# GG1991/macroc

Measured on AMD Instinct MI355X. Metric: Newton-iter DOF/s (assembly+CG) at 256^3 grid per GPU; SpMV achieved HBM GB/s, higher is better.
Workload: dtype f64

## Files before the change

### include/macroc_amd.h

```cpp
#ifndef MACROC_AMD_H
#define MACROC_AMD_H

#include <stddef.h>
#include <stdint.h>

#ifdef __cplusplus
extern "C" {
#endif

#define MCX_COMM_ID_BYTES 128

#define MCX_ABI_VERSION 3

enum { MCX_BC_BENDING = 0, MCX_BC_CIRCLE = 1 };

enum {
  MCX_KSP_CONVERGED_ITERATING = 0,
  MCX_KSP_CONVERGED_RTOL = 2,
  MCX_KSP_CONVERGED_ATOL = 3,
  MCX_KSP_DIVERGED_ITS = -3,
  MCX_KSP_DIVERGED_DTOL = -4,
  MCX_KSP_DIVERGED_INDEFINITE_PC = -8,
  MCX_KSP_DIVERGED_NANORINF = -9,
  MCX_KSP_DIVERGED_INDEFINITE_MAT = -10
// ... 56 lines not shown
  int64_t vi_exc_nodes;
  int64_t split_escapes;
  int64_t st_listed;
} mcx_info;

typedef struct {
  double strains_ms, homogenize_ms, residual_ms, jacobian_ms, solve_ms, update_ms;
  int64_t spmv_launches;
  double spmv_ms_total;
  int64_t spmv_bytes_per_launch;
  int64_t cg_vec_bytes_per_iter;
} mcx_timing;

const char* mcx_last_error(void);
const char* mcx_version(void);
int mcx_abi_version(void);

void mcx_default_opts(mcx_opts* o);
int mcx_parse_args(mcx_opts* o, int argc, const char* const* argv);

int mcx_comm_unique_id(void* id );

int mcx_plan(const mcx_opts* o, int rank, int nranks, mcx_info* info);
int mcx_plan_halo(const mcx_opts* o, int rank, int nranks, int* nnbr, int* nbr_rank, int64_t* send_cnt,
                  int64_t* recv_cnt, int64_t* send_nat, int64_t* recv_nat, int64_t* nsend, int64_t* nrecv);

int mcx_init(const mcx_opts* o, int rank, int nranks, const void* comm_id, void** ctx);
int mcx_local_group_create(int nranks, int device, void** group);
int mcx_local_group_destroy(void* group);
int mcx_local_group_barrier(void* group, int rank);
int mcx_init_local(const mcx_opts* o, int rank, void* group, void** ctx);
int mcx_finalize(void* ctx);
int mcx_get_info(void* ctx, mcx_info* info);
int mcx_comm_info(void* ctx, int* comm_ranks, int* comm_rank, int* device);

int mcx_material_set(void* ctx, int id, double E, double nu, double Sy, double Ka, int type);

typedef struct {
  void (*set_strain3)(int gpi, double* strain);
  void (*homogenize)(void);
  void (*get_stress3)(int gpi, double* stress);
  void (*get_ctan3)(int gpi, double* ctan);
  void (*update_vars)(void);
  int (*get_non_linear_gps)(void);
  double (*get_f_trial_max)(void);
} mcx_micropp_api;

typedef struct {
  int64_t nelem;
  int64_t ngp;
  const double* eps;
  double* sig;
  double* ctan;
  void* stream;
} mcx_gp_batch;

typedef struct {
  int (*homogenize)(void* user, const mcx_gp_batch* batch);
  int (*update_vars)(void* user);
  int (*nonlinear_stats)(void* user, int64_t* n_nonlinear, double* f_trial_max);
  void* user;
} mcx_device_law;

int mcx_set_micropp(void* ctx, const mcx_micropp_api* api);
int mcx_set_device_law(void* ctx, const mcx_device_law* law);
int mcx_set_gp_stress(void* ctx, const double* host );
// ... 58 lines not shown
```

### macroc_amd/__init__.py

```python
import ctypes as C
import os

import numpy as np

_HERE = os.path.dirname(os.path.abspath(__file__))
LIB_PATH = os.path.join(_HERE, "libmacroc_amd.so")
COMM_ID_BYTES = 128
ABI_VERSION = 3

BC_BENDING, BC_CIRCLE = 0, 1
KSP_REASONS = {2: "CONVERGED_RTOL", 3: "CONVERGED_ATOL", -3: "DIVERGED_ITS", -4: "DIVERGED_DTOL",
               -8: "DIVERGED_INDEFINITE_PC", -9: "DIVERGED_NANORINF", -10: "DIVERGED_INDEFINITE_MAT"}

EXPORTS = [
    "mcx_last_error", "mcx_version", "mcx_abi_version", "mcx_comm_info", "mcx_default_opts", "mcx_parse_args", "mcx_comm_unique_id", "mcx_plan", "mcx_plan_halo", "mcx_init",
    "mcx_local_group_create", "mcx_local_group_destroy", "mcx_local_group_barrier", "mcx_init_local",
    "mcx_finalize", "mcx_get_info", "mcx_material_set", "mcx_get_displacement", "mcx_zero_u", "mcx_apply_bc_u",
    "mcx_set_strains", "mcx_homogenize", "mcx_assembly_res", "mcx_assembly_jac", "mcx_solve", "mcx_update_u", "mcx_update_vars",
    "mcx_get_nonlinear_stats", "mcx_reduce_nonlinear", "mcx_calc_force", "mcx_write_vtu",
    "mcx_time_step", "mcx_get_u", "mcx_set_u", "mcx_get_b", "mcx_get_du", "mcx_get_strain", "mcx_get_stress",
    "mcx_owned_dofs", "mcx_dump_csr", "mcx_dump_dirichlet", "mcx_spmv", "mcx_get_ksp_history",
    "mcx_set_timing", "mcx_get_timing", "mcx_synchronize", "mcx_set_option", "mcx_time_spmv",
    "mcx_set_micropp", "mcx_set_device_law", "mcx_set_gp_stress", "mcx_set_gp_ctan", "mcx_get_gp_strain",
    "mcx_micro_get_ctan", "mcx_micro_get_phase",
    "mcx_get_gp_ctan", "mcx_micro_nl_get_info", "mcx_micro_nl_get_pool", "mcx_apply_args",
    "mcx_pc_apply", "mcx_pc_mg_info", "mcx_pc_mg_dump_csr",
]

LAWS = {"elastic": 0, "plastic": 1, "external": 2, "micro": 3, "micro_nl": 4}


class Opts(C.Structure):
    _fields_ = [
        ("NX", C.c_int64), ("NY", C.c_int64), ("NZ", C.c_int64),
        ("px", C.c_int), ("py", C.c_int), ("pz", C.c_int),
        ("lx", C.c_double), ("ly", C.c_double), ("lz", C.c_double),
        ("dt", C.c_double), ("final_time", C.c_double),
        ("ts", C.c_int), ("vtu_freq", C.c_int), ("bc_type", C.c_int), ("rad", C.c_double),
        ("newton_max_its", C.c_int), ("newton_min_tol", C.c_double), ("newton_rel_tol", C.c_double),
        ("ksp_rtol", C.c_double), ("ksp_abstol", C.c_double), ("ksp_dtol", C.c_double),
        ("ksp_max_it", C.c_int), ("micro_n", C.c_int), ("micro_type", C.c_int),
        ("micro_mat_1", C.c_double * 4), ("micro_mat_2", C.c_double * 4),
        ("device", C.c_int), ("ksp_monitor", C.c_int), ("mat_type", C.c_int), ("mat_law", C.c_int),
        ("mat_aij_split", C.c_int),
        ("mat_aij_vi", C.c_int),
        ("mat_vi_fma", C.c_int),
    ]


class Info(C.Structure):
    _fields_ = [
        ("NX", C.c_int64), ("NY", C.c_int64), ("NZ", C.c_int64),
        ("px", C.c_int), ("py", C.c_int), ("pz", C.c_int), ("rank", C.c_int), ("nranks", C.c_int),
        ("xs", C.c_int64), ("ys", C.c_int64), ("zs", C.c_int64), ("nx", C.c_int64), ("ny", C.c_int64), ("nz", C.c_int64),
        ("Xs", C.c_int64), ("Ys", C.c_int64), ("Zs", C.c_int64), ("Nx", C.c_int64), ("Ny", C.c_int64), ("Nz", C.c_int64),
        ("ndofs_global", C.c_int64), ("ndofs_local", C.c_int64), ("dof_offset", C.c_int64),
        ("nnz_local", C.c_int64), ("nnz_global", C.c_int64), ("nelem_local", C.c_int64), ("nelem_ext", C.c_int64),
        ("dx", C.c_double), ("dy", C.c_double), ("dz", C.c_double), ("wg", C.c_double),
        ("device_bytes", C.c_int64), ("device", C.c_int), ("storage", C.c_int), ("split_slots", C.c_int),
# ... 43 lines not shown

_LIB = None


class MacrocError(RuntimeError):
    pass


def lib():
    global _LIB
    if _LIB is not None:
        return _LIB
    if not os.path.exists(LIB_PATH):
        raise MacrocError(f"{LIB_PATH} not built: run `make` (or __graft_entry__.build())")
    L = C.CDLL(LIB_PATH)
    if L.mcx_abi_version() != ABI_VERSION:
        raise MacrocError(f"{LIB_PATH}: ABI {L.mcx_abi_version()}, this mirror needs {ABI_VERSION}: rebuild (`make`)")
    vp, d, i64 = C.c_void_p, C.POINTER(C.c_double), C.POINTER(C.c_int64)
    L.mcx_last_error.restype = C.c_char_p
    L.mcx_version.restype = C.c_char_p
    L.mcx_default_opts.argtypes = [C.POINTER(Opts)]
    L.mcx_parse_args.argtypes = [C.POINTER(Opts), C.c_int, C.POINTER(C.c_char_p)]
    L.mcx_comm_unique_id.argtypes = [C.c_void_p]
    L.mcx_init.argtypes = [C.POINTER(Opts), C.c_int, C.c_int, C.c_void_p, C.POINTER(C.c_void_p)]
    L.mcx_plan.argtypes = [C.POINTER(Opts), C.c_int, C.c_int, C.POINTER(Info)]
    L.mcx_plan_halo.argtypes = [C.POINTER(Opts), C.c_int, C.c_int, C.POINTER(C.c_int), C.POINTER(C.c_int),
                                i64, i64, i64, i64, i64, i64]
    L.mcx_local_group_create.argtypes = [C.c_int, C.c_int, C.POINTER(C.c_void_p)]
    L.mcx_local_group_destroy.argtypes = [vp]
    L.mcx_local_group_barrier.argtypes = [vp, C.c_int]
    L.mcx_init_local.argtypes = [C.POINTER(Opts), C.c_int, vp, C.POINTER(C.c_void_p)]
    L.mcx_finalize.argtypes = [vp]
    L.mcx_get_info.argtypes = [vp, C.POINTER(Info)]
    L.mcx_comm_info.argtypes = [vp, C.POINTER(C.c_int), C.POINTER(C.c_int), C.POINTER(C.c_int)]
    L.mcx_material_set.argtypes = [vp, C.c_int, C.c_double, C.c_double, C.c_double, C.c_double, C.c_int]
    L.mcx_get_displacement.argtypes = [vp, C.c_int]
    L.mcx_get_displacement.restype = C.c_double
    L.mcx_apply_bc_u.argtypes = [vp, C.c_double]
    for fn in ("mcx_zero_u", "mcx_set_strains", "mcx_homogenize", "mcx_assembly_jac", "mcx_update_u",
               "mcx_synchronize", "mcx_update_vars"):
        getattr(L, fn).argtypes = [vp]
    L.mcx_assembly_res.argtypes = [vp, d]
    L.mcx_solve.argtypes = [vp, C.POINTER(C.c_int), d, C.POINTER(C.c_int)]
    L.mcx_time_step.argtypes = [vp, C.c_int, C.POINTER(C.c_int), d, C.POINTER(C.c_int), d]
    for fn in ("mcx_get_u", "mcx_set_u", "mcx_get_b", "mcx_get_du", "mcx_get_strain", "mcx_get_stress"):
        getattr(L, fn).argtypes = [vp, d]
    L.mcx_owned_dofs.argtypes = [vp, i64, i64]
    L.mcx_get_nonlinear_stats.argtypes = [vp, i64, d]
    L.mcx_reduce_nonlinear.argtypes = [vp, i64, i64, d]
    L.mcx_calc_force.argtypes = [vp, d]
    L.mcx_write_vtu.argtypes = [vp, C.c_char_p]
    L.mcx_dump_csr.argtypes = [vp, i64, i64, d]
    L.mcx_dump_dirichlet.argtypes = [vp, i64, i64]
    L.mcx_spmv.argtypes = [vp, d, d]
    L.mcx_get_ksp_history.argtypes = [vp, d, i64]
    L.mcx_set_timing.argtypes = [vp, C.c_int]
    L.mcx_get_timing.argtypes = [vp, C.POINTER(Timing)]
    L.mcx_set_option.argtypes = [vp, C.c_char_p, C.c_double]
    L.mcx_apply_args.argtypes = [vp, C.c_int, C.POINTER(C.c_char_p)]
    L.mcx_time_spmv.argtypes = [vp, C.c_int, d]
    L.mcx_set_micropp.argtypes = [vp, C.POINTER(MicroppApi)]
    L.mcx_set_device_law.argtypes = [vp, C.POINTER(DeviceLaw)]
    ip = C.POINTER(C.c_int)
    L.mcx_micro_nl_get_info.argtypes = [vp, ip, ip, ip, d]
    L.mcx_micro_nl_get_pool.argtypes = [vp, i64, i64, i64]
    for fn in ("mcx_set_gp_stress", "mcx_set_gp_ctan", "mcx_get_gp_strain", "mcx_get_gp_ctan"):
# ... 132 lines not shown

    def apply_bc_on_u(self, U):
        _check(lib().mcx_apply_bc_u(self._ctx, float(U)), "apply_bc_on_u")

    def set_strains(self):
        _check(lib().mcx_set_strains(self._ctx), "set_strains")

    def homogenize(self):
        _check(lib().mcx_homogenize(self._ctx), "micropp_C_homogenize")

    def material_set(self, mid, E, nu, Sy=1e4, Ka=1e7, typ=1):
        _check(lib().mcx_material_set(self._ctx, mid, E, nu, Sy, Ka, typ), "micropp_C_material_set")

    def assembly_res(self):
        nrm = C.c_double()
        _check(lib().mcx_assembly_res(self._ctx, C.byref(nrm)), "assembly_res")
        return nrm.value

    def assembly_jac(self):
        _check(lib().mcx_assembly_jac(self._ctx), "assembly_jac")

    def solve_Ax(self):
        its, rn, reason = C.c_int(), C.c_double(), C.c_int()
        _check(lib().mcx_solve(self._ctx, C.byref(its), C.byref(rn), C.byref(reason)), "solve_Ax")
        return its.value, rn.value, reason.value

    def update_u(self):
        _check(lib().mcx_update_u(self._ctx), "VecAXPY(u,1,du)")

    def update_vars(self):
        _check(lib().mcx_update_vars(self._ctx), "micropp_C_update_vars")

    def get_info(self):
        inf = Info()
        _check(lib().mcx_get_info(self._ctx, C.byref(inf)), "mcx_get_info")
        return inf.as_dict()

    def comm_info(self):
        n, r, d = C.c_int(), C.c_int(), C.c_int()
        _check(lib().mcx_comm_info(self._ctx, C.byref(n), C.byref(r), C.byref(d)), "mcx_comm_info")
        return n.value, r.value, d.value

    def nonlinear_stats(self):
        n, f = C.c_int64(), C.c_double()
        _check(lib().mcx_get_nonlinear_stats(self._ctx, C.byref(n), C.byref(f)), "nonlinear_stats")
        return n.value, f.value

    def reduce_nonlinear(self):
        nl, nt, f = C.c_int64(), C.c_int64(), C.c_double()
        _check(lib().mcx_reduce_nonlinear(self._ctx, C.byref(nl), C.byref(nt), C.byref(f)), "reduce_nonlinear")
        return nl.value, nt.value, f.value

    def write_vtu(self, prefix):
        _check(lib().mcx_write_vtu(self._ctx, str(prefix).encode()), "write_vtu")

    def calc_force(self):
        f = C.c_double()
        _check(lib().mcx_calc_force(self._ctx, C.byref(f)), "calc_force")
        return f.value

    def time_step(self, time_s):
        k = max(self.opts.newton_max_its, 1)
        nits = C.c_int()
        res, kr = np.zeros(k), np.zeros(k)
        ki = (C.c_int * k)()
        _check(lib().mcx_time_step(self._ctx, int(time_s), C.byref(nits), _dp(res), ki, _dp(kr)), "time_step")
        n = nits.value
        return dict(newton_its=n, res=res[: n + 1 if n < k else n].tolist(), ksp_its=list(ki)[:n],
                    ksp_rnorm=kr[:n].tolist())
# ... 163 lines not shown
```

### macroc_amd/csrc/api.cpp

```cpp
#include <algorithm>
#include <cmath>
#include <cstdio>
#include <cstdlib>
#include <cstring>
#include <string>
#include <unordered_map>
#include <vector>

#include "mcx_internal.h"

namespace mcx {

static thread_local std::string g_err;
void set_error(const std::string& s) { g_err = s; }

int exc_return(const char* fn, const char* what) {
  try {
    g_err = std::string(fn) + ": internal exception: " + what;
  } catch (...) {
  }
  return MCX_EXC;
}

static const std::string g_test_throw = [] {
// ... 579 lines not shown
  }
  in->nelem_local = cnt[0] * cnt[1] * cnt[2];
  in->nelem_ext = g.nelem;
  in->dx = g.dx;
  in->dy = c.dy;
  in->dz = g.dz;
  in->wg = g.wg;
  in->device_bytes = c.device_bytes;
  in->device = c.device;
  in->storage = c.fmt;
  in->split_slots = c.fmt == FMT_SPLIT ? c.dsl.L : 0;
  in->split_bits = c.fmt == FMT_SPLIT ? (c.dsl.wide ? 32 : 16) : 0;
  in->vi_values = c.fmt == FMT_VI ? c.vi_n : 0;
  in->vi_bits = c.fmt == FMT_VI ? c.vi_bits : 0;
  in->vi_blocks = c.fmt == FMT_VI && c.vi_block ? c.vi_nblocks : 0;
  in->vi_exc_nodes = c.fmt == FMT_VI && c.vi_block ? c.vi_nexc : 0;
  in->split_escapes = c.fmt == FMT_SPLIT && c.dsl.esc ? c.dsl.nesc : 0;
  in->st_listed = c.device >= 0 && st_used(c) ? c.st_n : -1;
  if (c.device >= 0) spmv_tile(c, &in->spmv_tx, &in->spmv_ty, &in->spmv_kc);
  in->ex0 = g.ex0;
  in->ey0 = g.ey0;
  in->ez0 = g.ez0;
  in->nex = g.nex;
  in->ney = g.ney;
  in->nez = g.nez;
}


int mcx_get_info(void* ctx, mcx_info* in) try {
  MCX_ENTRY();
  GUARD(ctx);
  CTX(ctx);
  fill_info(c, in);
  return 0;
} MCX_CATCH

int mcx_comm_info(void* ctx, int* comm_ranks, int* comm_rank, int* device) try {
  MCX_ENTRY();
  GUARD(ctx);
  CTX(ctx);
  int n = 1, r = 0, d = c.device;
  if (c.lg) {
    n = c.lg->nranks;
    r = c.rank;
  } else if (int rc = comm_query(c, &n, &r, &d)) {
    return rc;
  }
  if (comm_ranks) *comm_ranks = n;
  if (comm_rank) *comm_rank = r;
  if (device) *device = d;
  return 0;
} MCX_CATCH

int mcx_plan(const mcx_opts* o, int rank, int nranks, mcx_info* in) try {
  MCX_ENTRY();
  if (!o || !in || nranks < 1 || rank < 0 || rank >= nranks) {
    set_error("mcx_plan: bad arguments");
    return 1;
  }
  Ctx c;
  c.o = *o;
  c.rank = rank;
  c.nranks = nranks;
  c.device = -1;
  int rc = setup_decomposition(c);
  if (rc) return rc;
// ... 1557 lines not shown
      set_error("vi_st_faces: partials buffer too small");
      return (c.st_ok || c.st_pending) && build_st(c) ? 1 : 2;
    }
    return 0;
  }
  if (!std::strcmp(name, "vi_st_pair")) {
    const int old = c.vi_st_pair;
    c.vi_st_pair = value != 0.;
    if (!partials_fit(c)) {
      c.vi_st_pair = old;
      set_error("vi_st_pair: partials buffer too small");
      return 2;
    }
    return 0;
  }
  if (!std::strcmp(name, "vi_st_fstream")) {
    c.vi_st_fstream = value != 0.;
    return 0;
  }
  if (!std::strcmp(name, "vi_st_l16")) {
    if (!(value == -1. || value == 0. || value == 1.)) {
      set_error("vi_st_l16: -1 (by the list's length), 0 or 1");
      return 1;
    }
    const int old = c.vi_st_l16;
    c.vi_st_l16 = (int)value;
    if (!partials_fit(c)) {
      c.vi_st_l16 = old;
      set_error("vi_st_l16: partials buffer too small");
      return 2;
    }
    return 0;
  }
  if (!std::strcmp(name, "vi_st_pf")) {
    if (!(value == 1. || value == 2. || value == 3.)) {
      set_error("vi_st_pf: 1 or 2");
      return 1;
    }
    c.vi_st_pf = (int)value;
    return 0;
  }
  if (!std::strcmp(name, "vi_st_ty")) {
    if (!(value == 8. || value == 16.)) {
      set_error("vi_st_ty: 8 or 16");
      return 1;
    }
    const int old = c.vi_st_ty;
    c.vi_st_ty = (int)value;
    if (!partials_fit(c)) {
      c.vi_st_ty = old;
      set_error("vi_st_ty: partials buffer too small");
      return 2;
    }
    return 0;
  }
  if (!std::strcmp(name, "vi_st_tail")) {
    const int old = c.vi_st_tail;
    c.vi_st_tail = value != 0.;
    if (!partials_fit(c)) {
      c.vi_st_tail = old;
      set_error("vi_st_tail: partials buffer too small");
      return 2;
    }
    return 0;
  }
  if (!std::strcmp(name, "vi_st")) {
// ... 224 lines not shown
```

### macroc_amd/csrc/kernels.hip

```cpp
#include <algorithm>
#include <cstring>
#include <cmath>

#include "mcx_internal.h"

namespace mcx {

__constant__ double cB[8][6][24];

static constexpr int TPB = 256;

__device__ __forceinline__ void node_ijk(const Geo& g, int n, int& i, int& j, int& k) {
  i = n % g.nx;
  int t = n / g.nx;
  j = t % g.ny;
  k = t / g.ny;
}

__device__ __forceinline__ int pad_of(const Geo& g, int i, int j, int k) {
  return (i + 1) + (j + 1) * g.PX + (k + 1) * g.PX * g.PY;
}

__device__ __forceinline__ int u_of(const Geo& g, int i, int j, int k) {
  return 64 + i + (j + 1) * g.UX + (k + 1) * g.UXY;
}

__host__ __device__ inline int dirichlet_mask(const Geo& g, int gi, int gj, int gk) {
  if (g.bc_type == MCX_BC_CIRCLE) {
    if (gj == 0 && (gi == 0 || gi == g.NX - 1 || gk == 0 || gk == g.NZ - 1)) return 7;
    if (gj == g.NY - 1) {
      double x = g.lx / 2. - ((double)gi * g.dx + g.dx / 2.);
      double z = g.lz / 2. - ((double)gk * g.dz + g.dz / 2.);
      if ((x * x + z * z) < (g.rad * g.rad)) return 2;
    }
    return 0;
  }
  if (g.bc_type == MCX_BC_BENDING) return (gi == 0 || gi == g.NX - 1) ? 7 : 0;
// ... 4210 lines not shown
    if (more && !NOSTAGE) {
      __syncthreads();
#pragma unroll
      for (int m = 0; m < NL; m++) {
        const int e = me + m * T;
        if (e < PLANE) {
          xs[(k + 3 - k0 + 1) & 3][e] = PF2 ? cur[0][m] : xr[0][m];
          xs[(k + 4 - k0 + 1) & 3][e] = PF2 ? cur[1][m] : xr[1][m];
        }
      }
      __syncthreads();
    }
  };
  if (PF2) {
    for (int k = k0; k < k1; k += 4) {
      step(k, pfa, pfb);
      if (k + 2 < k1) step(k + 2, pfb, pfa);
    }
  } else {
    for (int k = k0; k < k1; k += 2) step(k, pfa, pfb);
  }
  if (TAIL) {
    __syncthreads();
    st_faces(g, sf, coef, slot, x, y, dot, &xs[0][0]);
    st_tail<T>(g, list, (int64_t)b * cnt / gridDim.x, (int64_t)(b + 1) * cnt / gridDim.x, I, bdict, exc, x, y,
               reinterpret_cast<double2*>(&xs[0][0]), dot);
  }
  if (DOT) {
    const double s = block_sum<T>(dot, sh);
    if (threadIdx.x == 0) part[blockIdx.x] = s;
  }
}

template <bool DOT, bool GATED, bool L16 = true>
__global__ __launch_bounds__(SFP_T) void k_spmv_face(Geo g, StFaces sf, const double* __restrict__ coef,
                                                   const unsigned* __restrict__ slot, const double* __restrict__ x,
                                                   double* __restrict__ y, double* __restrict__ part,
                                                   const CgState* __restrict__ cg, const int* __restrict__ list,
                                                   int64_t cnt, const u32x4* __restrict__ I,
                                                   const double* __restrict__ bdict, const double* __restrict__ exc,
                                                   int nd = VI_MAX) {
  static_assert(SFP_N >= VI_MAX * VIB_STRIDE, "the dictionary fits the patch's LDS");
  __shared__ __attribute__((aligned(16))) double S[SFP_N];
  __shared__ double sh[SFP_T / 64];
  if (GATED && cg->reason) return;
  double dot = 0.;
  constexpr int LPB = L16 ? SFP_T / ST16 : SFP_T;
  const int64_t NLB = (cnt + LPB - 1) / LPB;
  if ((int64_t)blockIdx.x >= NLB) {
    const SfPatch q = sf_patch(g, sf, blockIdx.x - NLB);
    sf_stage(g, q, x, S, threadIdx.x);
    __syncthreads();
    sf_rows(g, q, coef, slot, S, y, dot, threadIdx.x);
  } else {
    const int64_t lo = (int64_t)blockIdx.x * LPB;
    if (L16) st_tail16<SFP_T>(g, list, lo, min(cnt, lo + LPB), I, bdict, exc, x, y, reinterpret_cast<double2*>(S), dot, nd);
    else st_tail<SFP_T>(g, list, lo, min(cnt, lo + LPB), I, bdict, exc, x, y, reinterpret_cast<double2*>(S), dot, nd);
  }
  if (DOT) {
    const double sm = block_sum<SFP_T>(dot, sh);
    if (threadIdx.x == 0) part[blockIdx.x] = sm;
  }
}

constexpr int SP_RLP = 198;

// ... 1537 lines not shown
  return (face_enum(c.g).n + TPB - 1) / TPB;
}

bool fusep(const Ctx& c);
bool st_fusep(const Ctx& c);

static bool st_auto(const Ctx& c) {
  return c.g.nown >= ST_MIN_NODES || (c.vi_nexc > 0 && c.vi_nexc * 10 <= (int64_t)c.g.nown);
}

bool st_used(const Ctx& c) {
  int tx, ty;
  vis_shape(c, tx, ty);
  return st_wanted(c) && c.st_ok && c.fmt == FMT_VI && c.vi_block && vi_staged(c) && c.vi_fma && c.vi_uni && c.vi_patch &&
         tx == 64 && (!fusep(c) || st_fusep(c));
}

bool st_fusep(const Ctx& c) { return c.vi_st_pair && !c.vi_st_tail; }

static bool sp_used(const Ctx& c) { return st_used(c) && c.vi_st_pair && !c.vi_st_tail; }

static ZTiling sp_tiling(const Ctx& c) {
  const int ty = c.vi_st_ty;
  ZTiling t;
  t.ntx = (c.g.nx + 63) / 64;
  t.nty = (c.g.ny + ty - 1) / ty;
  const int tiles = t.ntx * t.nty, want = c.spmv_zblocks > 0 ? c.spmv_zblocks : c.g.ncu * (16 / ty);
  t.nzc = std::max(1, std::min(c.g.nz, (want + tiles - 1) / tiles));
  t.kc = (c.g.nz + t.nzc - 1) / t.nzc;
  t.nzc = (c.g.nz + t.kc - 1) / t.kc;
  return t;
}

static bool st_l16(const Ctx& c) {
  return c.vi_st_l16 > 0 || (c.vi_st_l16 < 0 && (int64_t)ST16 * c.st_n * 2 <= (int64_t)c.g.ncu * 1024);
}

static int64_t stface_blocks(const Ctx& c) {
  const int lpb = st_l16(c) ? SFP_T / ST16 : SFP_T;
  return st_used(c) && !c.vi_st_tail ? c.st_faces.u[6] + (c.st_n + lpb - 1) / lpb : 0;
}

static int64_t exc_blocks(const Ctx& c) {
  if (!(c.fmt == FMT_VI && c.vi_block && c.vi_nexc && vi_staged(c) && c.vi_exc_kernel) || st_used(c)) return 0;
  return (c.vi_nexc + TPB - 1) / TPB;
}

int64_t spmv_nparts(const Ctx& c) {
  if (c.fmt == FMT_SPLIT && c.dsl.dense) return node_blocks(c);
  return spmv_grid_blocks(c) + faces_blocks(c) + exc_blocks(c) + stface_blocks(c);
}

bool partials_fit(const Ctx& c) {
  return std::max(spmv_nparts(c), node_blocks(c)) + 32 <= c.partials_cap / 2;
}

bool st_wanted(const Ctx& c) { return c.vi_st == 1 || (c.vi_st < 0 && st_auto(c)); }

int upload_constants(Ctx& c) {
  double B[8][6][24];
  compute_B_table(B);
  MCX_HIP(hipMemcpyToSymbol(HIP_SYMBOL(cB), B, sizeof(B)));
  return 0;
}

void launch_apply_bc_u(Ctx& c, double U) {
// ... 792 lines not shown
    }
  return true;
}

template <bool DV, bool GV, int D>
static void sp_dbg1(Ctx& c, int nb, const double* xpad, double* y, const ZTiling& zt) {
  if (c.vi_st_ty == 16)
    hipLaunchKernelGGL((k_spmv_sp<DV, GV, 16, false, D>), dim3(nb), dim3(1024), 0, c.stream, c.g, c.st_coef,
                       c.st_mask, c.st_npx, c.st_npy, xpad, y, c.partials, c.cg, zt);
  else
    hipLaunchKernelGGL((k_spmv_sp<DV, GV, 8, false, D>), dim3(nb), dim3(512), 0, c.stream, c.g, c.st_coef,
                       c.st_mask, c.st_npx, c.st_npy, xpad, y, c.partials, c.cg, zt);
}
template <bool DV, bool GV>
static void sp_dbg(Ctx& c, int nb, const double* xpad, double* y, const ZTiling& zt) {
  switch (zt.dbg) {
    case 1: sp_dbg1<DV, GV, 1>(c, nb, xpad, y, zt); break;
    case 2: sp_dbg1<DV, GV, 2>(c, nb, xpad, y, zt); break;
    case 3: sp_dbg1<DV, GV, 3>(c, nb, xpad, y, zt); break;
    case 4: sp_dbg1<DV, GV, 4>(c, nb, xpad, y, zt); break;
    case 8: sp_dbg1<DV, GV, 8>(c, nb, xpad, y, zt); break;
    case 12: sp_dbg1<DV, GV, 12>(c, nb, xpad, y, zt); break;
    case 44: sp_dbg1<DV, GV, 44>(c, nb, xpad, y, zt); break;
    case 1024: sp_dbg1<DV, GV, 1024>(c, nb, xpad, y, zt); break;
    case 36: sp_dbg1<DV, GV, 36>(c, nb, xpad, y, zt); break;
    case 40: sp_dbg1<DV, GV, 40>(c, nb, xpad, y, zt); break;
    case 32: sp_dbg1<DV, GV, 32>(c, nb, xpad, y, zt); break;
    case 35: sp_dbg1<DV, GV, 35>(c, nb, xpad, y, zt); break;
    default: sp_dbg1<DV, GV, 0>(c, nb, xpad, y, zt); break;
  }
}

void launch_spmv(Ctx& c, const double* xpad, double* y, bool dot, bool gated) {
  const int nb = (int)spmv_grid_blocks(c);
  const SpmvTiling tl = spmv_tiling(c.g, c.spmv_subl);
  if (c.fmt == FMT_VI && c.vi_block) {
    const u32x4* I = reinterpret_cast<const u32x4*>(c.vi_idx);
    if (vi_staged(c)) {
      ZTiling zt = vis_tiling(c);
      zt.dbg = c.split_dbg;
      zt.wmap = c.vi_wmap;
      zt.xlist = c.vi_exc_list;
      zt.xskip = exc_blocks(c) > 0;
      zt.ypair = c.vi_ypair && (c.g.nx % 2) == 0;
      int tx, ty;
      vis_shape(c, tx, ty);
      if (st_used(c)) {
        if (sp_used(c)) {
          const int dbg = zt.dbg;
          zt = sp_tiling(c);
          zt.dbg = dbg;
        }
        StFaces sfv = c.st_faces;
        int64_t stn = c.st_n, nbfa = stface_blocks(c);
        if (c.face_dbg && nbfa) {
          if (c.face_dbg & 1) stn = 0;
          if (c.face_dbg & 2) {
            const int64_t d = sfv.u[2];
            for (int q = 1; q < 7; q++) sfv.u[q] = std::max<int64_t>(0, sfv.u[q] - d);
          }
          if (c.face_dbg & 4)
            for (int q = 3; q < 7; q++) sfv.u[q] = sfv.u[2];
          const int lpb = st_l16(c) ? SFP_T / ST16 : SFP_T;
          nbfa = sfv.u[6] + (stn + lpb - 1) / lpb;
        }
        double* pf = c.partials + nb;
        const int ndict = c.vi_nblocks > 0 ? c.vi_nblocks : VI_MAX;
#define MCX_SP_DBG(DV, GV) sp_dbg<DV, GV>(c, nb, xpad, y, zt)
#define MCX_ST(DV, GV)                                                                                             \
  do {                                                                                                            \
    const bool fs = nbfa && !c.vi_st_tail && fstream_ok(c);        \
    hipStream_t fst = fs ? c.f_stream : c.stream;                                                                 \
    if (fs) (void)hipEventRecord(c.ev_fx, c.stream);                                                              \
    if (c.vi_st_tail)                                                                                             \
      hipLaunchKernelGGL((k_spmv_st<DV, GV, true>), dim3(nb), dim3(1024), 0, c.stream, c.g, c.st_coef, c.st_mask,   \
                         c.st_npx, c.st_npy, xpad, y, c.partials, c.cg, zt, c.st_list, c.st_n, I, c.vi_bdict,     \
                         c.vi_exc, c.st_slot, c.st_faces);                                                        \
    else if (c.vi_st_pair && zt.dbg > 0)                                                                        \
      MCX_SP_DBG(DV, GV);                                                                                         \
    else if (c.vi_st_pair && c.vi_st_ty == 16)                                                                    \
      hipLaunchKernelGGL((k_spmv_sp<DV, GV, 16>), dim3(nb), dim3(1024), 0, c.stream, c.g, c.st_coef, c.st_mask,     \
                         c.st_npx, c.st_npy, xpad, y, c.partials, c.cg, zt);                                      \
    else if (c.vi_st_pair)                                                                                        \
      hipLaunchKernelGGL((k_spmv_sp<DV, GV, 8>), dim3(nb), dim3(512), 0, c.stream, c.g, c.st_coef, c.st_mask,       \
                         c.st_npx, c.st_npy, xpad, y, c.partials, c.cg, zt);                                      \
    else if (c.vi_st_pf == 3)                                                                                     \
      hipLaunchKernelGGL((k_spmv_st<DV, GV, false, false, true>), dim3(nb), dim3(1024), 0, c.stream, c.g,            \
                         c.st_coef, c.st_mask, c.st_npx, c.st_npy, xpad, y, c.partials, c.cg, zt);                \
    else if (c.vi_st_pf == 2)                                                                                     \
      hipLaunchKernelGGL((k_spmv_st<DV, GV, false, true>), dim3(nb), dim3(1024), 0, c.stream, c.g, c.st_coef,       \
                         c.st_mask, c.st_npx, c.st_npy, xpad, y, c.partials, c.cg, zt);                           \
    else                                                                                                          \
      hipLaunchKernelGGL((k_spmv_st<DV, GV>), dim3(nb), dim3(1024), 0, c.stream, c.g, c.st_coef, c.st_mask,         \
                         c.st_npx, c.st_npy, xpad, y, c.partials, c.cg, zt);                                      \
    if (fs) (void)hipStreamWaitEvent(fst, c.ev_fx, 0);                                                            \
    if (nbfa && st_l16(c))                                                                                        \
      hipLaunchKernelGGL((k_spmv_face<DV, GV>), dim3((unsigned)nbfa), dim3(SFP_T), 0, fst, c.g, sfv,                \
                         c.st_coef, c.st_slot, xpad, y, pf, c.cg, c.st_list, stn, I, c.vi_bdict, c.vi_exc, ndict); \
    else if (nbfa)                                                                                                \
      hipLaunchKernelGGL((k_spmv_face<DV, GV, false>), dim3((unsigned)nbfa), dim3(SFP_T), 0, fst, c.g,              \
                         sfv, c.st_coef, c.st_slot, xpad, y, pf, c.cg, c.st_list, stn, I, c.vi_bdict,   \
                         c.vi_exc, ndict);                                                                        \
    if (fs) {                                                                                                     \
      (void)hipEventRecord(c.ev_fd, fst);                                                                         \
      (void)hipStreamWaitEvent(c.stream, c.ev_fd, 0);                                                             \
    }                                                                                                             \
  } while (0)
        if (dot && gated) MCX_ST(true, true);
        else if (dot) MCX_ST(true, false);
        else MCX_ST(false, false);
#undef MCX_ST
#undef MCX_SP_DBG
        return;
      }
#define MCX_VIBM(TXV, TYV, XVV, UV, PV, ...)                                                                          \
  do {                                                                                                             \
    if (dot && gated)                                                                                              \
      hipLaunchKernelGGL((k_spmv_vibm<true, true, TXV, TYV, XVV, UV, PV, ##__VA_ARGS__>), dim3(nb), dim3(1024), 0,        \
                         c.stream, c.g, I, c.vi_bdict, xpad, y, c.partials, c.cg, zt);                             \
    else if (dot)                                                                                                  \
      hipLaunchKernelGGL((k_spmv_vibm<true, false, TXV, TYV, XVV, UV, PV, ##__VA_ARGS__>), dim3(nb), dim3(1024), 0,       \
                         c.stream, c.g, I, c.vi_bdict, xpad, y, c.partials, c.cg, zt);                             \
    else                                                                                                           \
      hipLaunchKernelGGL((k_spmv_vibm<false, false, TXV, TYV, XVV, UV, PV, ##__VA_ARGS__>), dim3(nb), dim3(1024), 0,      \
// ... 829 lines not shown
```

### macroc_amd/csrc/mcx_internal.h

```cpp
#pragma once

#include <hip/hip_runtime.h>

#include <cstdint>
#include <string>
#include <vector>

#include "../../include/macroc_amd.h"

namespace mcx {

constexpr int NGP = 8, NPE = 8, NVOI = 6;
constexpr int NSLOT = 243;
constexpr int NPAIR = 122;
constexpr int GROUP = 64;
constexpr int USLOT = 123;
constexpr int UPAIR = 62;

void set_error(const std::string& s);

struct Geo {
  int NX, NY, NZ;
  int xs, ys, zs;
  int nx, ny, nz;
// ... 252 lines not shown
  double* h_vib_dict = nullptr;
  int vib_onepass = 1;
  unsigned char* elem_plain = nullptr;
  double* cref = nullptr;
  unsigned* vi_xslot = nullptr;
  int* vi_xlist = nullptr;
  unsigned* vi_xcnt = nullptr;
  double* vi_exc = nullptr;
  int64_t vi_exc_bytes = 0;
  int64_t vi_nexc = 0;
  bool plain_ke = false;
  int vi_exc_max = 300;
  double* ke_uni = nullptr;
  int aij_vi = 1;
  int vi_fma = 1;
  int vi_patch = 1;
  int vi_ring3 = 0;
  int vi_exc_list = VI_EXC_LIST;
  int vi_wmap = 1;
  int vi_tx = 0;
  int vi_uni = 1;
  int vi_ypair = 0;
  int cg_ublocks = 0;
  int vi_lg = 2;
  int cg_p2d = 0;
  int vi_lg_exc = 1;
  int vi_st = -1;
  int vi_st_faces = 1;
  int vi_st_l16 = -1;
  int vi_st_pf = 1;
  int vi_st_ty = 16;
  int vi_st_pair = 0;
  int vi_st_tail = 0;
  double* st_coef = nullptr;
  unsigned* st_ids = nullptr;
  unsigned* st_slot = nullptr;
  int* st_list = nullptr;
  unsigned* st_cnt = nullptr;
  unsigned long long* st_mask = nullptr;
  int64_t st_mask_bytes = 0, st_n = 0;
  int st_npx = 0, st_npy = 0;
  bool st_ok = false;
  bool st_pending = false;
  unsigned st_fm = 0;
  StFaces st_faces = {};
  int vi_exc_kernel = 1;
  int vi_wdesc = 1;
  unsigned* wd = nullptr;
  int64_t wd_bytes = 0;
  bool wd_ok = false;
  int wd_npx = 0, wd_npy = 0;
  int64_t wd_blocks_fma = 0, wd_blocks_exact = 0, wd_blocks_two = 0;
  int vi_xread = 1;
  int vi_stage = -1;
  bool vi_declined = false;
  int fmt = FMT_V;
  bool assembled = false;
  int aij_split = 1;
  int split_maxq = 4;
  int split_dense = 1;
  bool split_declined = false;
  int split_dbg = 0;
  int face_dbg = 0;
  int split_wide = 0;
  int split_tx = 0;
  int split_ty = 0;
// ... 211 lines not shown
```

Baseline: 22.35 million.

## Stage stencil SpMV x-planes into LDS via buffer-load-to-LDS DMA ring

Adds a variant of the structured-stencil SpMV kernel that uses buffer_load ... lds (direct global-to-LDS loads) to fill a 5-slot ring of staged x planes. Two z-planes are processed per iteration with prefetch of upcoming planes, so x loads skip VGPRs and overlap with FMA work. The variant is picked by default when eligibility checks on padding alignment, PX parity and option settings pass, and it is exposed through a query function. The cost is heavier LDS use (close to the 160KB limit) and extra barriers, which may lower occupancy.

```diff
diff --git a/include/macroc_amd.h b/include/macroc_amd.h
--- a/include/macroc_amd.h
+++ b/include/macroc_amd.h
@@ -112,6 +112,7 @@
 int mcx_init_local(const mcx_opts* o, int rank, void* group, void** ctx);
 int mcx_finalize(void* ctx);
 int mcx_get_info(void* ctx, mcx_info* info);
+int mcx_get_st_dma(void* ctx, int* on);
 int mcx_comm_info(void* ctx, int* comm_ranks, int* comm_rank, int* device);
 
 int mcx_material_set(void* ctx, int id, double E, double nu, double Sy, double Ka, int type);
diff --git a/macroc_amd/__init__.py b/macroc_amd/__init__.py
--- a/macroc_amd/__init__.py
+++ b/macroc_amd/__init__.py
@@ -24,7 +24,7 @@
     "mcx_set_micropp", "mcx_set_device_law", "mcx_set_gp_stress", "mcx_set_gp_ctan", "mcx_get_gp_strain",
     "mcx_micro_get_ctan", "mcx_micro_get_phase",
     "mcx_get_gp_ctan", "mcx_micro_nl_get_info", "mcx_micro_nl_get_pool", "mcx_apply_args",
-    "mcx_pc_apply", "mcx_pc_mg_info", "mcx_pc_mg_dump_csr",
+    "mcx_pc_apply", "mcx_pc_mg_info", "mcx_pc_mg_dump_csr", "mcx_get_st_dma",
 ]
 
 LAWS = {"elastic": 0, "plastic": 1, "external": 2, "micro": 3, "micro_nl": 4}
@@ -134,6 +134,7 @@
     L.mcx_init_local.argtypes = [C.POINTER(Opts), C.c_int, vp, C.POINTER(C.c_void_p)]
     L.mcx_finalize.argtypes = [vp]
     L.mcx_get_info.argtypes = [vp, C.POINTER(Info)]
+    L.mcx_get_st_dma.argtypes = [vp, C.POINTER(C.c_int)]
     L.mcx_comm_info.argtypes = [vp, C.POINTER(C.c_int), C.POINTER(C.c_int), C.POINTER(C.c_int)]
     L.mcx_material_set.argtypes = [vp, C.c_int, C.c_double, C.c_double, C.c_double, C.c_double, C.c_int]
     L.mcx_get_displacement.argtypes = [vp, C.c_int]
@@ -332,9 +333,10 @@
         _check(lib().mcx_update_vars(self._ctx), "micropp_C_update_vars")
 
     def get_info(self):
-        inf = Info()
+        inf, on = Info(), C.c_int()
         _check(lib().mcx_get_info(self._ctx, C.byref(inf)), "mcx_get_info")
-        return inf.as_dict()
+        _check(lib().mcx_get_st_dma(self._ctx, C.byref(on)), "mcx_get_st_dma")
+        return dict(inf.as_dict(), st_dma=on.value)
 
     def comm_info(self):
         n, r, d = C.c_int(), C.c_int(), C.c_int()
diff --git a/macroc_amd/csrc/api.cpp b/macroc_amd/csrc/api.cpp
--- a/macroc_amd/csrc/api.cpp
+++ b/macroc_amd/csrc/api.cpp
@@ -635,6 +635,14 @@
   GUARD(ctx);
   CTX(ctx);
   fill_info(c, in);
+  return 0;
+} MCX_CATCH
+
+int mcx_get_st_dma(void* ctx, int* on) try {
+  MCX_ENTRY();
+  GUARD(ctx);
+  CTX(ctx);
+  if (on) *on = c.st_dma_last;
   return 0;
 } MCX_CATCH
 
@@ -2258,6 +2266,14 @@
     }
     return 0;
   }
+  if (!std::strcmp(name, "vi_st_dma")) {
+    if (!(value == -1. || value == 0. || value == 1.)) {
+      set_error("vi_st_dma: -1 (where eligible), 0 or 1");
+      return 1;
+    }
+    c.vi_st_dma = (int)value;
+    return 0;
+  }
   if (!std::strcmp(name, "vi_st_pf")) {
     if (!(value == 1. || value == 2. || value == 3.)) {
       set_error("vi_st_pf: 1 or 2");
diff --git a/macroc_amd/csrc/kernels.hip b/macroc_amd/csrc/kernels.hip
--- a/macroc_amd/csrc/kernels.hip
+++ b/macroc_amd/csrc/kernels.hip
@@ -3,6 +3,7 @@
 #include <cmath>
 
 #include "mcx_internal.h"
+#include "st_dma_map.h"
 
 namespace mcx {
 
@@ -4279,6 +4280,155 @@
   }
 }
 
+typedef __attribute__((address_space(3))) void st_lds_void;
+__device__ __forceinline__ void st_dma16(__amdgpu_buffer_rsrc_t r, double* dst, unsigned voff) {
+  __builtin_amdgcn_raw_ptr_buffer_load_lds(r, (st_lds_void*)dst, 16, voff, 0, 0, 0);
+}
+
+template <bool DOT, bool GATED>
+__global__ __launch_bounds__(1024) void k_spmv_st_dma(Geo g, const double* __restrict__ coef,
+                                                      const unsigned long long* __restrict__ mask, int npx, int npy,
+                                                      const double* __restrict__ x, double* __restrict__ y,
+                                                      double* __restrict__ part, const CgState* __restrict__ cg,
+                                                      ZTiling zt, int sft) {
+  constexpr int TX = ST_DMA_TX, TY = ST_DMA_TY, T = TX * TY, RL = ST_DMA_RL, SLOT = ST_DMA_SLOT, NS = ST_DMA_SLOTS;
+  static_assert(RL == vibm_rl<TX, true>() && T == 64 * ST_DMA_WAVES, "k_spmv_st's staged plane");
+  constexpr int S9 = NS * SLOT, SH = S9 + 27, NLDS = SH + T / 64;
+  static_assert(NLDS * sizeof(double) <= 160 * 1024, "the 5-slot ring fits a CU's LDS");
+  __shared__ __attribute__((aligned(16))) double L[NLDS];
+  if (GATED && cg->reason) return;
+  const int b = blockIdx.x;
+  const int xcd = b & 7, t8 = b >> 3;
+  const int slab = (zt.nty + 7) >> 3;
+  const int ty0 = xcd * slab;
+  const int nty_here = min(slab, zt.nty - ty0);
+  const int per = max(nty_here, 0) * zt.ntx * zt.nzc;
+  const int me = threadIdx.x;
+  double dot = 0.;
+  if (t8 >= per) {
+    if (DOT) {
+      const double s = block_sum<T>(dot, &L[SH]);
+      if (threadIdx.x == 0) part[blockIdx.x] = s;
+    }
+    return;
+  }
+  const int txi = t8 % zt.ntx, r8 = t8 / zt.ntx;
+  const int tyi = ty0 + r8 % nty_here, zc = r8 / nty_here;
+  const int i0 = txi * TX, j0 = tyi * TY;
+  const int k0 = zc * zt.kc, k1 = min(g.nz, k0 + zt.kc);
+  const int wv = __builtin_amdgcn_readfirstlane(me >> 6), ln = me & 63;
+  if (me < 27) L[S9 + me] = coef[me * VIB_STRIDE + 8];
+  const int px = wv & 3, py = wv >> 2;
+  const int lx = px * 16 + (ln & 15), ly = py * 4 + (ln >> 4);
+  const int i = i0 + lx, j = j0 + ly;
+  const bool inxy = i < g.nx && j < g.ny;
+  const int PX = g.PX, PXY = g.PX * g.PY;
+  const int gpx = __builtin_amdgcn_readfirstlane((i0 >> 4) + px), gpy = __builtin_amdgcn_readfirstlane((j0 >> 2) + py);
+  const bool wvin = gpx < npx && gpy < npy;
+  const int len = 3 * min(TX + 2, g.nx + 2 - i0);
+  const int rows = min(TY + 2, g.ny + 2 - j0);
+  const int pc0 = st_dma_piece(wv, 0), pc1 = st_dma_piece(wv, 1);
+  const bool has1 = st_dma_piece_ok(pc1);
+  const unsigned src0 = st_dma_src(pc0, ln, i0, j0, PX, len, rows, sft);
+  const unsigned src1 = has1 ? st_dma_src(pc1, ln, i0, j0, PX, len, rows, sft) : ST_DMA_OOB;
+  auto dma = [&](int p, int so) {
+    const __amdgpu_buffer_rsrc_t rx = sp_rsrc(x + (int64_t)(p + 1) * PXY * 3 - st_dma_rec_lead(sft) / 8,
+                                              p > g.nz ? 0 : st_dma_rec_bytes(PXY, sft));
+    st_dma16(rx, &L[so + st_dma_dst(pc0)], src0);
+    if (has1) st_dma16(rx, &L[so + st_dma_dst(pc1)], src1);
+  };
+#pragma unroll
+  for (int s = 0; s < 4; s++) dma(k0 - 1 + s, s * SLOT);
+  asm volatile("s_waitcnt vmcnt(0)" ::: "memory");
+  __syncthreads();
+  typedef const volatile __attribute__((address_space(3))) double lds_vdouble;
+  lds_vdouble* xsv = (lds_vdouble*)&L[0];
+  const int lb = st_dma_read0(lx, ly, sft);
+  int s0 = 0;
+  auto nxt = [&](int so) { return so + SLOT == NS * SLOT ? 0 : so + SLOT; };
+  for (int k = k0; k < k1; k += 2) {
+    const bool two = k + 1 < k1, more = k + 2 < k1;
+    const int s1 = nxt(s0), s2 = nxt(s1), s3 = nxt(s2), s4 = nxt(s3);
+    if (more) dma(k + 3, s4);
+    unsigned long long m0 = ~0ull, m1 = ~0ull;
+    if (wvin) {
+      m0 = mask[((int64_t)k * npy + gpy) * npx + gpx];
+      if (two) m1 = mask[((int64_t)(k + 1) * npy + gpy) * npx + gpx];
+    }
+    double ya0 = 0., ya1 = 0., ya2 = 0., yb0 = 0., yb1 = 0., yb2 = 0.;
+    double ca0 = 0., ca1 = 0., ca2 = 0., cb0 = 0., cb1 = 0., cb2 = 0.;
+    int sa = s0, sb = s1, ry = lb;
+#pragma unroll 1
+    for (int g9 = 0; g9 < 9; g9++) {
+      double av[27], xa[9], xb[9];
+#pragma unroll
+      for (int t = 0; t < 3; t++) {
+#pragma unroll
+        for (int q = 0; q < 8; q++) av[t * 9 + q] = coef[(g9 * 3 + t) * VIB_STRIDE + q];
+        av[t * 9 + 8] = L[S9 + g9 * 3 + t];
+      }
+      const int ra = sa + ry, rb = sb + ry;
+#pragma unroll
+      for (int q = 0; q < 9; q++) {
+        xa[q] = xsv[ra + q];
+        xb[q] = xsv[rb + q];
+      }
+      __builtin_amdgcn_sched_barrier(0);
+      if (g9 == 4) {
+        ca0 = xa[3], ca1 = xa[4], ca2 = xa[5];
+        cb0 = xb[3], cb1 = xb[4], cb2 = xb[5];
+      }
+#pragma unroll
+      for (int t = 0; t < 3; t++) {
+#pragma unroll
+        for (int q = 0; q < 9; q++) {
+          const int r = q / 3, cc = q % 3;
+          const double a = av[t * 9 + q];
+          double& ya = r == 0 ? ya0 : (r == 1 ? ya1 : ya2);
+          double& yb = r == 0 ? yb0 : (r == 1 ? yb1 : yb2);
+          ya = __builtin_fma(a, xa[3 * t + cc], ya);
+          yb = __builtin_fma(a, xb[3 * t + cc], yb);
+        }
+      }
+      __builtin_amdgcn_sched_barrier(0);
+      ry += RL;
+      if (g9 == 2 || g9 == 5) {
+        ry = lb;
+        sa = sb;
+        sb = nxt(sb);
+      }
+      if (g9 == 2) {
+        asm volatile("s_waitcnt lgkmcnt(0)" ::: "memory");
+        __builtin_amdgcn_s_barrier();
+        if (more) dma(k + 4, s0);
+      }
+    }
+    asm volatile("s_waitcnt vmcnt(0) lgkmcnt(0)" ::: "memory");
+    {
+      const bool la = inxy && !((m0 >> ln) & 1ull), lb2 = two && inxy && !((m1 >> ln) & 1ull);
+      const int64_t pls = 3 * (int64_t)g.nx * g.ny;
+      const __amdgpu_buffer_rsrc_t ra = sp_rsrc(y + pls * k, pls * 8), rb = sp_rsrc(y + pls * min(k + 1, g.nz - 1), pls * 8);
+      const unsigned o = 24u * (unsigned)(i + g.nx * j), oa = la ? o : SP_OOB, ob = lb2 ? o : SP_OOB;
+      typedef unsigned u32x2v __attribute__((ext_vector_type(2)));
+      __builtin_amdgcn_raw_buffer_store_b64(__builtin_bit_cast(u32x2v, ya0), ra, oa, 0, 2);
+      __builtin_amdgcn_raw_buffer_store_b64(__builtin_bit_cast(u32x2v, ya1), ra, oa + 8, 0, 2);
+      __builtin_amdgcn_raw_buffer_store_b64(__builtin_bit_cast(u32x2v, ya2), ra, oa + 16, 0, 2);
+      __builtin_amdgcn_raw_buffer_store_b64(__builtin_bit_cast(u32x2v, yb0), rb, ob, 0, 2);
+      __builtin_amdgcn_raw_buffer_store_b64(__builtin_bit_cast(u32x2v, yb1), rb, ob + 8, 0, 2);
+      __builtin_amdgcn_raw_buffer_store_b64(__builtin_bit_cast(u32x2v, yb2), rb, ob + 16, 0, 2);
+      if (DOT && la) dot += ca0 * ya0 + ca1 * ya1 + ca2 * ya2;
+      if (DOT && lb2) dot += cb0 * yb0 + cb1 * yb1 + cb2 * yb2;
+    }
+    __builtin_amdgcn_s_barrier();
+    s0 = s2;
+    (void)s3;
+  }
+  if (DOT) {
+    const double s = block_sum<T>(dot, &L[SH]);
+    if (threadIdx.x == 0) part[blockIdx.x] = s;
+  }
+}
+
 template <bool DOT, bool GATED, bool L16 = true>
 __global__ __launch_bounds__(SFP_T) void k_spmv_face(Geo g, StFaces sf, const double* __restrict__ coef,
                                                    const unsigned* __restrict__ slot, const double* __restrict__ x,
@@ -5882,6 +6032,13 @@
   return t;
 }
 
+static int st_dma_sft(const Ctx& c) { return (c.pad_off / 8) & 1; }
+static bool st_dma_ok(const Ctx& c, const double* xpad) {
+  return c.vi_st_dma != 0 && st_used(c) && !c.vi_st_pair && !c.vi_st_tail && c.vi_st_pf == 1 && c.g.PX % 2 == 0 &&
+         c.pad_off % 8 == 0 && c.pad_off >= 0 && c.pad_off <= 240 &&
+         (reinterpret_cast<uintptr_t>(xpad) - (uintptr_t)c.pad_off) % 16 == 0;
+}
+
 static bool st_l16(const Ctx& c) {
   return c.vi_st_l16 > 0 || (c.vi_st_l16 < 0 && (int64_t)ST16 * c.st_n * 2 <= (int64_t)c.g.ncu * 1024);
 }
@@ -6740,6 +6897,7 @@
 }
 
 void launch_spmv(Ctx& c, const double* xpad, double* y, bool dot, bool gated) {
+  c.st_dma_last = 0;
   const int nb = (int)spmv_grid_blocks(c);
   const SpmvTiling tl = spmv_tiling(c.g, c.spmv_subl);
   if (c.fmt == FMT_VI && c.vi_block) {
@@ -6798,6 +6956,9 @@
     else if (c.vi_st_pf == 2)                                                                                     \
       hipLaunchKernelGGL((k_spmv_st<DV, GV, false, true>), dim3(nb), dim3(1024), 0, c.stream, c.g, c.st_coef,       \
                          c.st_mask, c.st_npx, c.st_npy, xpad, y, c.partials, c.cg, zt);                           \
+    else if ((c.st_dma_last = st_dma_ok(c, xpad)))                                                                \
+      hipLaunchKernelGGL((k_spmv_st_dma<DV, GV>), dim3(nb), dim3(1024), 0, c.stream, c.g, c.st_coef, c.st_mask,     \
+                         c.st_npx, c.st_npy, xpad, y, c.partials, c.cg, zt, st_dma_sft(c));                       \
     else                                                                                                          \
       hipLaunchKernelGGL((k_spmv_st<DV, GV>), dim3(nb), dim3(1024), 0, c.stream, c.g, c.st_coef, c.st_mask,         \
                          c.st_npx, c.st_npy, xpad, y, c.partials, c.cg, zt);                                      \
diff --git a/macroc_amd/csrc/mcx_internal.h b/macroc_amd/csrc/mcx_internal.h
--- a/macroc_amd/csrc/mcx_internal.h
+++ b/macroc_amd/csrc/mcx_internal.h
@@ -308,6 +308,8 @@
   int vi_st_ty = 16;
   int vi_st_pair = 0;
   int vi_st_tail = 0;
+  int vi_st_dma = -1;
+  int st_dma_last = 0;
   double* st_coef = nullptr;
   unsigned* st_ids = nullptr;
   unsigned* st_slot = nullptr;
diff --git a/macroc_amd/csrc/st_dma_map.h b/macroc_amd/csrc/st_dma_map.h
--- /dev/null
+++ b/macroc_amd/csrc/st_dma_map.h
@@ -0,0 +1,38 @@
+#pragma once
+
+#if defined(__HIPCC__) || defined(__CUDACC__)
+#define ST_DMA_HD __host__ __device__
+#else
+#define ST_DMA_HD
+#endif
+
+constexpr int ST_DMA_TX = 64, ST_DMA_TY = 16;
+constexpr int ST_DMA_RL = 208, ST_DMA_PR = ST_DMA_TY + 2;
+constexpr int ST_DMA_PLANE = ST_DMA_PR * ST_DMA_RL;
+constexpr int ST_DMA_PIECE = 128;
+constexpr int ST_DMA_NPIECE = (ST_DMA_PLANE + ST_DMA_PIECE - 1) / ST_DMA_PIECE;
+constexpr int ST_DMA_SLOT = ST_DMA_NPIECE * ST_DMA_PIECE;
+constexpr int ST_DMA_SLOTS = 5;
+constexpr int ST_DMA_WAVES = 16;
+constexpr unsigned ST_DMA_OOB = 0x80000000u;
+static_assert(ST_DMA_RL % 2 == 0, "an element pair never straddles a staged row");
+static_assert(3 * (ST_DMA_TX + 2) + 1 <= ST_DMA_RL, "a shifted row fits the staged row");
+static_assert(ST_DMA_NPIECE <= 2 * ST_DMA_WAVES, "two pieces per wave cover a plane");
+
+ST_DMA_HD inline int st_dma_piece(int wave, int m) { return wave + ST_DMA_WAVES * m; }
+ST_DMA_HD inline bool st_dma_piece_ok(int piece) { return piece < ST_DMA_NPIECE; }
+
+ST_DMA_HD inline int st_dma_dst(int piece) { return ST_DMA_PIECE * piece; }
+
+ST_DMA_HD inline unsigned st_dma_src(int piece, int lane, int i0, int j0, int PX, int len, int rows, int sft) {
+  const int e = ST_DMA_PIECE * piece + 2 * lane;
+  const int rr = e / ST_DMA_RL, q = e - rr * ST_DMA_RL;
+  return e >= ST_DMA_PLANE || q >= len + sft || rr >= rows ? ST_DMA_OOB : 8u * (unsigned)(3 * (i0 + (j0 + rr) * PX) + q);
+}
+
+ST_DMA_HD inline int st_dma_rec_lead(int sft) { return 8 * sft; }
+ST_DMA_HD inline long long st_dma_rec_bytes(long long PXY, int sft) { return 24 * PXY + 16 * sft; }
+
+ST_DMA_HD inline int st_dma_read0(int lx, int ly, int sft) { return ly * ST_DMA_RL + 3 * lx + sft; }
+
+ST_DMA_HD inline int st_dma_slot(int p, int k0) { return (p - k0 + 1) % ST_DMA_SLOTS; }
```

After: 22.76 million (median of 6 runs). 1.02x the previous value.
